# SajayR/TRIAD

Measured on AMD Instinct MI355X. Metric: tri-modal triples/sec (whole node) + loss parity, B=256 at 1/2/4/8 MI355X, higher is better.
Workload: dtype bf16

## Files before the change

include/triad_hip.h:

```cpp
#ifndef TRIAD_HIP_H
#define TRIAD_HIP_H

#include <hip/hip_runtime_api.h>

#ifdef __cplusplus
extern "C" {
#endif

#define TRIAD_EINVAL 1001

int triad_pairsim_nparts(int R_pad, int Bk);

int triad_pairsim_fwd(const void* Q, const void* K, int R, int R_pad, int Nq, int Bq, int Bk, int Nk_pad,
                      int Nk_eff, int D, const float* temp, float clamp_lo, int diag, int diag_off,
                      float* rowmax, int* argmax, double* nn_part, float* diagS, void* dS, long long CT,
                      double* st_part, const int* k_len, hipStream_t stream);

typedef struct triad_pairsim_problem {
  const void* Q;
  const void* K;
  int R, R_pad, Nq, Bq, Bk, Nk_pad, Nk_eff;
  const float* temp;
  float clamp_lo;
  int diag, diag_off;
// ... 161 lines not shown
                   hipStream_t stream);

long long triad_conv0_dw_workspace_bytes(int B, int T, int C);
int triad_conv0_dw(const void* wave, long long Lp, const void* dy0, int B, int T, int Tp, int C, void* ws, float* dw0,
                   hipStream_t stream);

int triad_posconv(const void* x, const void* wt, const float* bias, void* y, int B, int T, int C, int groups,
                  int pad, hipStream_t stream);

long long triad_posconv_dw_part_bytes(int C, int groups, int splits);
int triad_posconv_dw(const void* x, const void* dy, int B, int T, int C, int groups, int pad, int splits, float* part,
                     hipStream_t stream);

int triad_attn_fwd(const void* q, long long q_sB, long long q_sN, const void* k, long long k_sB, long long k_sN,
                   const void* v, long long v_sB, long long v_sN, int B, int H, int N, int D, float scale, void* out,
                   long long out_sB, long long out_sN, float* lse, hipStream_t stream);
int triad_attn_bwd(const void* q, long long q_sB, long long q_sN, const void* k, long long k_sB, long long k_sN,
                   const void* v, long long v_sB, long long v_sN, const void* o, long long o_sB, long long o_sN,
                   const void* dout, long long do_sB, long long do_sN, const float* lse, int B, int H, int N, int D,
                   float scale, void* dq, long long dq_sB, long long dq_sN, void* dk, long long dk_sB,
                   long long dk_sN, void* dv, long long dv_sB, long long dv_sN, float* delta, hipStream_t stream);
int triad_attn_dropmask(int B, int H, int N, float p, unsigned seed, unsigned* wq, unsigned* wk, hipStream_t stream);
int triad_attn_fwd_dropout(const void* q, long long q_sB, long long q_sN, const void* k, long long k_sB,
                           long long k_sN, const void* v, long long v_sB, long long v_sN, int B, int H, int N, int D,
                           float scale, const unsigned* wq, float p, void* out, long long out_sB, long long out_sN,
                           float* lse, hipStream_t stream);
int triad_attn_bwd_dropout(const void* q, long long q_sB, long long q_sN, const void* k, long long k_sB,
                           long long k_sN, const void* v, long long v_sB, long long v_sN, const void* o,
                           long long o_sB, long long o_sN, const void* dout, long long do_sB, long long do_sN,
                           const float* lse, int B, int H, int N, int D, float scale, const unsigned* wq,
                           const unsigned* wk, float p, void* dq, long long dq_sB, long long dq_sN, void* dk,
                           long long dk_sB, long long dk_sN, void* dv, long long dv_sB, long long dv_sN, float* delta,
                           hipStream_t stream);

int triad_attn_long_dropmask(int B, int H, int N, float p, unsigned seed, unsigned* wq, unsigned* wk,
                             hipStream_t stream);
int triad_attn_long_fwd(const void* q, long long q_sB, long long q_sN, const void* k, long long k_sB, long long k_sN,
                        const void* v, long long v_sB, long long v_sN, int B, int H, int N, int D, float scale,
                        const unsigned* wq, float p, void* out, long long out_sB, long long out_sN, float* lse,
                        hipStream_t stream);
int triad_attn_long_bwd(const void* q, long long q_sB, long long q_sN, const void* k, long long k_sB, long long k_sN,
                        const void* v, long long v_sB, long long v_sN, const void* o, long long o_sB, long long o_sN,
                        const void* dout, long long do_sB, long long do_sN, const float* lse, int B, int H, int N,
                        int D, float scale, const unsigned* wq, const unsigned* wk, float p, void* dq, long long dq_sB,
                        long long dq_sN, void* dk, long long dk_sB, long long dk_sN, void* dv, long long dv_sB,
                        long long dv_sN, float* delta, hipStream_t stream);

int triad_rows_nt(const void* X, long long ldx, int M, int K, const void* W, int J, void* out, hipStream_t stream);
int triad_lora_update(void* Y, long long ldy, int M, int O, const void* T, const void* Bs, hipStream_t stream);
int triad_lora_tn_blocks(int M);
int triad_lora_tn(const void* Y, long long ldy, int M, int O, const void* T, const void* Wt, void* dt, float alpha,
                  float* slabs, float* out, hipStream_t stream);

int triad_addln_fwd(const float* x, const void* y, const float* g, const float* w, const float* b, float eps, int M,
                    int D, float* xn, void* ln, int out_f32, float* mean, float* rstd, hipStream_t stream);
int triad_addln_bwd(const void* dln, int dln_f32, const float* dres, const float* xn, const float* mean,
                    const float* rstd, const float* w, const float* g, int M, int D, float* dx, void* dy,
                    hipStream_t stream);

int triad_dropaddln_fwd(const float* res, const void* y, const float* w, const float* b, float eps, int M, int D,
                        float p, unsigned seed, float* h, void* hb, float* mean, float* rstd, hipStream_t stream);
int triad_dropaddln_bwd_blocks(int M);
int triad_dropaddln_bwd(const float* dh, const void* dhb, const float* res, const void* y, const float* mean,
                        const float* rstd, const float* w, int M, int D, float p, unsigned seed, float* dres, void* dy,
                        float* part, hipStream_t stream);
long long triad_gelu_table_bytes(void);
// ... 23 lines not shown
```

triad_amd/_lib.py:

```python
from __future__ import annotations

import ctypes as C
import os
import threading

_HERE = os.path.dirname(os.path.abspath(__file__))
DEFAULT_LIB = os.path.join(_HERE, "libtriad_hip.so")
LIB_PATH = os.environ.get("TRIAD_LIB_VARIANT", DEFAULT_LIB)

vp, i32, u32, i64, f32, f64 = C.c_void_p, C.c_int, C.c_uint, C.c_longlong, C.c_float, C.c_double

SIGNATURES = {
    "triad_pairsim_nparts": [i32, i32],
    "triad_pairsim_fwd": [vp, vp, i32, i32, i32, i32, i32, i32, i32, i32, vp, f32, i32, i32, vp, vp, vp, vp, vp,
                          i64, vp, vp, vp],
    "triad_pairsim_fwd_multi": [vp, i32, vp],
    "triad_pairsim_diag": [vp, i32, vp],
    "triad_clip_reduce": [vp, i32, i32, i32, i32, vp, vp, vp, vp],
    "triad_diag_smooth": [vp, i32, i32, i32, i32, f64, vp, vp, vp, vp],
    "triad_diag_sparsity": [vp, i32, i32, i32, i32, f32, f64, vp, vp, vp, vp],
    "triad_losshead": [vp, i32, i32, vp, vp, i32, f64, vp, i32, f64, f32, vp, vp, vp, vp],
    "triad_pairsim_dS": [vp, vp, i32, i32, i32, i32, i32, i32, i32, i32, vp, f32, i32, i32, vp, vp, vp, vp, vp,
                         vp, i64, vp, vp],
    "triad_split_pack": [vp, i32, i32, i32, i64, vp, vp, vp],
# ... 43 lines not shown
    "triad_chgn_gelu_fwd": [vp, i32, i32, i32, i32, vp, vp, f32, vp, vp, vp, vp, vp],
    "triad_chgn_gelu_bwd": [vp, vp, i32, i32, i32, i32, vp, vp, vp, vp, vp, vp, vp, vp, vp],
    "triad_gemm_bf16_form": [vp, i64, i32, vp, i64, i32, i32, i32, i32, vp, vp, i64, i32, i32, vp],
    "triad_gemm_w8_workgroups": [i32, i32],
    "triad_gemm_bf16_tiles": [vp, i64, i32, vp, i64, i32, i32, i32, i32, vp, vp, i64, i32, vp, i32, i32, vp],
    "triad_conv0_dw_workspace_bytes": [i32, i32, i32],
    "triad_conv0_dw": [vp, i64, vp, i32, i32, i32, i32, vp, vp, vp],
    "triad_c0gn_fwd": [vp, i64, vp, i32, i32, i32, i32, vp, vp, f32, vp, vp, vp, vp, vp, vp],
    "triad_posconv": [vp, vp, vp, vp, i32, i32, i32, i32, i32, vp],
    "triad_posconv_dw_part_bytes": [i32, i32, i32],
    "triad_posconv_dw": [vp, vp, i32, i32, i32, i32, i32, i32, vp, vp],
    "triad_rows_nt": [vp, i64, i32, i32, vp, i32, vp, vp],
    "triad_lora_update": [vp, i64, i32, i32, vp, vp, vp],
    "triad_dropaddln_fwd": [vp, vp, vp, vp, f32, i32, i32, f32, u32, vp, vp, vp, vp, vp],
    "triad_dropaddln_bwd_blocks": [i32],
    "triad_dropaddln_bwd": [vp, vp, vp, vp, vp, vp, vp, i32, i32, f32, u32, vp, vp, vp, vp],
    "triad_gelu_table_bytes": [],
    "triad_gelu_table": [vp, vp],
    "triad_geludrop_fwd": [vp, i64, f32, u32, vp, vp, vp],
    "triad_geludrop_bwd": [vp, vp, i64, f32, u32, vp, vp, vp],
    "triad_dropout_keep": [i64, f32, u32, vp, vp],
    "triad_addln_fwd": [vp, vp, vp, vp, vp, f32, i32, i32, vp, vp, i32, vp, vp, vp],
    "triad_addln_bwd": [vp, i32, vp, vp, vp, vp, vp, vp, i32, i32, vp, vp, vp],
    "triad_lora_tn_blocks": [i32],
    "triad_lora_tn": [vp, i64, i32, i32, vp, vp, vp, f32, vp, vp, vp],
    "triad_attn_dropmask": [i32, i32, i32, f32, u32, vp, vp, vp],
    "triad_attn_fwd_dropout": [vp, i64, i64, vp, i64, i64, vp, i64, i64, i32, i32, i32, i32, f32, vp, f32, vp, i64,
                               i64, vp, vp],
    "triad_attn_bwd_dropout": [vp, i64, i64, vp, i64, i64, vp, i64, i64, vp, i64, i64, vp, i64, i64, vp, i32, i32,
                               i32, i32, f32, vp, vp, f32, vp, i64, i64, vp, i64, i64, vp, i64, i64, vp, vp],
    "triad_attn_fwd": [vp, i64, i64, vp, i64, i64, vp, i64, i64, i32, i32, i32, i32, f32, vp, i64, i64, vp, vp],
    "triad_attn_bwd": [vp, i64, i64, vp, i64, i64, vp, i64, i64, vp, i64, i64, vp, i64, i64, vp, i32, i32, i32,
                       i32, f32, vp, i64, i64, vp, i64, i64, vp, i64, i64, vp, vp],
    "triad_attn_long_dropmask": [i32, i32, i32, f32, u32, vp, vp, vp],
    "triad_attn_long_fwd": [vp, i64, i64, vp, i64, i64, vp, i64, i64, i32, i32, i32, i32, f32, vp, f32, vp, i64, i64,
                            vp, vp],
    "triad_attn_long_bwd": [vp, i64, i64, vp, i64, i64, vp, i64, i64, vp, i64, i64, vp, i64, i64, vp, i32, i32, i32,
                            i32, f32, vp, vp, f32, vp, i64, i64, vp, i64, i64, vp, i64, i64, vp, vp],
    "triad_dense_nparts": [i64],
    "triad_dense_rowmax": [vp, i32, i32, i32, i32, i32, vp, vp, vp],
    "triad_nonneg_fwd": [vp, i64, f32, vp, vp],
    "triad_nonneg_bwd": [vp, i64, f32, f32, vp, vp, vp],
    "triad_sims_bwd_pack": [vp, vp, vp, vp, vp, i32, i32, i32, i32, i32, vp, vp, i64, vp, vp],
    "triad_sum_parts": [vp, i32, f64, vp, vp],
}
RESTYPES = {"triad_pairsim_nparts": C.c_int, "triad_chgn_workspace_bytes": C.c_longlong,
            "triad_conv0_dw_workspace_bytes": C.c_longlong, "triad_gelu_table_bytes": C.c_longlong,
            "triad_posconv_dw_part_bytes": C.c_longlong,
            "triad_lora_tn_blocks": C.c_int, "triad_dropaddln_bwd_blocks": C.c_int,
            "triad_colsum_splits": C.c_int, "triad_colsum_dma_splits": C.c_int, "triad_dense_nparts": C.c_int,
            "triad_rowpanel_count": C.c_int, "triad_gemm_w8_workgroups": C.c_int}

BACKBONE_ENTRY_POINTS = frozenset({
    "triad_chgn_gelu_fwd", "triad_chgn_gelu_bwd", "triad_gemm_bf16_form", "triad_gemm_bf16_tiles", "triad_conv0_dw",
    "triad_c0gn_fwd",
    "triad_posconv", "triad_posconv_dw", "triad_gemm_bf16_splitk", "triad_rows_nt", "triad_lora_update",
    "triad_dropaddln_fwd", "triad_dropaddln_bwd", "triad_gelu_table", "triad_geludrop_fwd", "triad_geludrop_bwd",
    "triad_dropout_keep", "triad_addln_fwd", "triad_addln_bwd", "triad_lora_tn", "triad_attn_dropmask",
    "triad_attn_fwd_dropout", "triad_attn_bwd_dropout", "triad_attn_fwd", "triad_attn_bwd",
    "triad_attn_long_dropmask", "triad_attn_long_fwd", "triad_attn_long_bwd"})


def hot_path_entry_points():
    return tuple(n for n in SIGNATURES if n not in RESTYPES and n not in BACKBONE_ENTRY_POINTS)



class PairsimProblem(C.Structure):
    _fields_ = [("Q", vp), ("K", vp), ("R", i32), ("R_pad", i32), ("Nq", i32), ("Bq", i32), ("Bk", i32),
                ("Nk_pad", i32), ("Nk_eff", i32), ("temp", vp), ("clamp_lo", f32), ("diag", i32), ("diag_off", i32),
                ("rowmax", vp), ("argmax", vp), ("nn_part", vp), ("diagS", vp), ("dS", vp), ("CT", i64),
                ("st_part", vp), ("k_tiles", vp)]


_lock = threading.Lock()
_lib = None


class TriadError(RuntimeError):
    pass


def load():
    global _lib
    with _lock:
        if _lib is None:
            if not os.path.exists(LIB_PATH):
                raise TriadError(f"{LIB_PATH} not found: build it with `python -m triad_amd.build` "
                                 "(or __graft_entry__.build()); there is no CPU fallback")
            if LIB_PATH == DEFAULT_LIB:
                _check_fresh()
            lib = C.CDLL(LIB_PATH)
            for name, args in SIGNATURES.items():
# ... 68 lines not shown
```

triad_amd/csrc/attention.hip:

```cpp
#include "attention_tiles.h"

namespace {

template <int NT>
__device__ __forceinline__ void load_rows2(char* l0, const bf16* b0, long long s0, char* l1, const bf16* b1,
                                           long long s1, int N) {
  static_assert((NT * 32 * 8) % 256 == 0, "256 threads");
  constexpr int PER = NT * 32 * 8 / 256;
  bf16x8 r0[PER], r1[PER];
#pragma unroll
  for (int i = 0; i < PER; ++i) {
    const int e = threadIdx.x + 256 * i, r = e >> 3, c = e & 7;
    r0[i] = r < N ? *(const bf16x8*)(b0 + (long long)r * s0 + c * 8) : (bf16x8){};
    r1[i] = r < N ? *(const bf16x8*)(b1 + (long long)r * s1 + c * 8) : (bf16x8){};
  }
#pragma unroll
  for (int i = 0; i < PER; ++i) {
    const int e = threadIdx.x + 256 * i, r = e >> 3, c = e & 7;
    const int off = r * 128 + ((c ^ swz(r)) << 4);
    *(bf16x8*)(l0 + off) = r0[i];
    *(bf16x8*)(l1 + off) = r1[i];
  }
}

template <int NKT, bool DROP>
__global__ __launch_bounds__(256, 2) void attn_fwd_kernel(AttnArgs a) {
  __shared__ __attribute__((aligned(16))) char lds[2 * NKT * 32 * 128];
  char* kl = lds;
  char* vl = lds + NKT * 32 * 128;
  const int bh = blockIdx.y, b = bh / a.H, hh = bh - b * a.H;
  const int lane = threadIdx.x & 63, wave = threadIdx.x >> 6, h = lane >> 5, ql = lane & 31;
  const int qt = blockIdx.x * 4 + wave;
  const int q = qt * 32 + ql;
  const bool qok = q < a.N;
  bf16x8 qf[4];
  {
    const bf16* qp = a.q + b * a.q_sB + (long long)(qok ? q : 0) * a.q_sN + hh * HD + 8 * h;
#pragma unroll
    for (int s = 0; s < 4; ++s) qf[s] = qok ? *(const bf16x8*)(qp + 16 * s) : (bf16x8){};
  }
  load_rows2<NKT>(kl, a.k + b * a.k_sB + hh * HD, a.k_sN, vl, a.v + b * a.v_sB + hh * HD, a.v_sN, a.N);
  __syncthreads();
  if (qt * 32 >= a.N) return;
  f32x16 acc[NKT];
#pragma unroll
  for (int kt = 0; kt < NKT; ++kt) {
    acc[kt] = (f32x16){};
#pragma unroll
    for (int s = 0; s < 4; ++s) acc[kt] = mfma32(lds_b128(kl, kt * 32 + ql, 2 * s + h), qf[s], acc[kt]);
  }
  const int nlast = a.N - (NKT - 1) * 32;
  if (nlast < 32) {
#pragma unroll
    for (int v = 0; v < 16; ++v)
      if (acc_row(v, h) >= nlast) acc[NKT - 1][v] = -INFINITY;
  }
  float m = -INFINITY;
#pragma unroll
  for (int kt = 0; kt < NKT; ++kt)
#pragma unroll
    for (int v = 0; v < 16; ++v) m = fmaxf(m, acc[kt][v]);
  m = fmaxf(m, __shfl_xor(m, 32));
  const float c2 = a.scale * LOG2E;
  const float mo = m * c2;
  float l = 0.f;
#pragma unroll
  for (int kt = 0; kt < NKT; ++kt)
#pragma unroll
    for (int v = 0; v < 16; ++v) {
      const float p = __builtin_amdgcn_exp2f(fmaf(acc[kt][v], c2, -mo));
      acc[kt][v] = p;
      l += p;
    }
  l += __shfl_xor(l, 32);
  if (DROP) {
#pragma unroll
    for (int kt = 0; kt < NKT; ++kt) {
      const unsigned w = qok ? a.wq[((long long)bh * a.N + q) * NKT + kt] : 0u;
#pragma unroll
      for (int v = 0; v < 16; ++v) acc[kt][v] = tile_bit(w, v, h) ? acc[kt][v] : 0.f;
    }
  }

  f32x16 o0 = {}, o1 = {};
#pragma unroll
  for (int kt = 0; kt < NKT; ++kt)
#pragma unroll
    for (int half = 0; half < 2; ++half) {
      const int c = 2 * kt + half;
      const bf16x8 pf = pack8(acc[kt], half);
      o0 = mfma32(frag_tr(vl, c, 0, lane), pf, o0);
      o1 = mfma32(frag_tr(vl, c, 32, lane), pf, o1);
    }
  if (!qok) return;
  const float inv = (DROP ? a.drop_scale : 1.f) / l;
  bf16* op = a.out + b * a.out_sB + (long long)q * a.out_sN + hh * HD;
  store_cols(op, o0, inv, h);
  store_cols(op + 32, o1, inv, h);
  if (h == 0) a.lse[(long long)bh * a.N + q] = m * a.scale + logf(l);
}

template <int NKT, bool DROP>
__global__ __launch_bounds__(256, 2) void attn_dq_kernel(AttnArgs a) {
  __shared__ __attribute__((aligned(16))) char lds[2 * NKT * 32 * 128];
  char* kl = lds;
  char* vl = lds + NKT * 32 * 128;
  const int bh = blockIdx.y, b = bh / a.H, hh = bh - b * a.H;
  const int lane = threadIdx.x & 63, wave = threadIdx.x >> 6, h = lane >> 5, ql = lane & 31;
  const int qt = blockIdx.x * 4 + wave;
  const int q = qt * 32 + ql;
  const bool qok = q < a.N;
  bf16x8 qf[4], df[4], ov[4];
  {
    const long long qq = qok ? q : 0;
    const bf16* qp = a.q + b * a.q_sB + qq * a.q_sN + hh * HD + 8 * h;
    const bf16* dp = a.dout + b * a.do_sB + qq * a.do_sN + hh * HD + 8 * h;
    const bf16* op = a.o + b * a.o_sB + qq * a.o_sN + hh * HD + 8 * h;
#pragma unroll
    for (int s = 0; s < 4; ++s) {
      qf[s] = qok ? *(const bf16x8*)(qp + 16 * s) : (bf16x8){};
      df[s] = qok ? *(const bf16x8*)(dp + 16 * s) : (bf16x8){};
      ov[s] = qok ? *(const bf16x8*)(op + 16 * s) : (bf16x8){};
    }
  }
  const float lse2 = qok ? a.lse[(long long)bh * a.N + q] * LOG2E : 0.f;
  load_rows2<NKT>(kl, a.k + b * a.k_sB + hh * HD, a.k_sN, vl, a.v + b * a.v_sB + hh * HD, a.v_sN, a.N);
  __syncthreads();
  if (qt * 32 >= a.N) return;
  float dl = 0.f;
#pragma unroll
  for (int s = 0; s < 4; ++s)
#pragma unroll
    for (int i = 0; i < 8; ++i) dl = fmaf((float)df[s][i], (float)ov[s][i], dl);
  dl += __shfl_xor(dl, 32);
  if (qok && h == 0) a.delta[(long long)bh * a.N + q] = dl;
  const float c2 = a.scale * LOG2E;
  f32x16 g0 = {}, g1 = {};
#pragma unroll
  for (int kt = 0; kt < NKT; ++kt) {
    f32x16 s = {}, dp = {};
#pragma unroll
    for (int st = 0; st < 4; ++st) {
      s = mfma32(lds_b128(kl, kt * 32 + ql, 2 * st + h), qf[st], s);
      dp = mfma32(lds_b128(vl, kt * 32 + ql, 2 * st + h), df[st], dp);
    }
    const int nv = a.N - kt * 32;
    const unsigned w = DROP && qok ? a.wq[((long long)bh * a.N + q) * NKT + kt] : 0u;
#pragma unroll
    for (int v = 0; v < 16; ++v) {
      const bool ok = qok && acc_row(v, h) < nv;
      const float e = __builtin_amdgcn_exp2f(fmaf(s[v], c2, -lse2));
      const float p = ok ? e : 0.f;
      const float dpv = DROP ? (tile_bit(w, v, h) ? dp[v] * a.drop_scale : 0.f) : dp[v];
      s[v] = p * (dpv - dl);
    }
#pragma unroll
    for (int half = 0; half < 2; ++half) {
      const int c = 2 * kt + half;
      const bf16x8 sf = pack8(s, half);
      g0 = mfma32(frag_tr(kl, c, 0, lane), sf, g0);
      g1 = mfma32(frag_tr(kl, c, 32, lane), sf, g1);
    }
  }
  if (!qok) return;
  bf16* gp = a.dq + b * a.dq_sB + (long long)q * a.dq_sN + hh * HD;
  store_cols(gp, g0, a.scale, h);
  store_cols(gp + 32, g1, a.scale, h);
}

template <int NQT, bool DROP>
__global__ __launch_bounds__(256, 2) void attn_dkv_kernel(AttnArgs a) {
  __shared__ __attribute__((aligned(16))) char lds[2 * NQT * 32 * 128];
  __shared__ float stat[2][NQT * 32];
  char* ql_ = lds;
  char* dl_ = lds + NQT * 32 * 128;
  const int bh = blockIdx.y, b = bh / a.H, hh = bh - b * a.H;
  const int lane = threadIdx.x & 63, wave = threadIdx.x >> 6, h = lane >> 5, kl = lane & 31;
  const int kt = blockIdx.x * 4 + wave;
  const int key = kt * 32 + kl;
  const bool kok = key < a.N;
  bf16x8 kf[4], vf[4];
  {
    const long long kk = kok ? key : 0;
    const bf16* kp = a.k + b * a.k_sB + kk * a.k_sN + hh * HD + 8 * h;
    const bf16* vp = a.v + b * a.v_sB + kk * a.v_sN + hh * HD + 8 * h;
#pragma unroll
    for (int s = 0; s < 4; ++s) {
      kf[s] = kok ? *(const bf16x8*)(kp + 16 * s) : (bf16x8){};
      vf[s] = kok ? *(const bf16x8*)(vp + 16 * s) : (bf16x8){};
    }
  }
  load_rows2<NQT>(ql_, a.q + b * a.q_sB + hh * HD, a.q_sN, dl_, a.dout + b * a.do_sB + hh * HD, a.do_sN, a.N);
  for (int i = threadIdx.x; i < NQT * 32; i += blockDim.x) {
    const bool ok = i < a.N;
    stat[0][i] = ok ? a.lse[(long long)bh * a.N + i] * LOG2E : INFINITY;
    stat[1][i] = ok ? a.delta[(long long)bh * a.N + i] : 0.f;
  }
  __syncthreads();
  if (kt * 32 >= a.N) return;
  const float c2 = a.scale * LOG2E;
  f32x16 dv0 = {}, dv1 = {}, dk0 = {}, dk1 = {};
#pragma unroll 1
  for (int qt = 0; qt < NQT; ++qt) {
    f32x16 s = {}, dp = {};
#pragma unroll
    for (int st = 0; st < 4; ++st) {
      s = mfma32(lds_b128(ql_, qt * 32 + kl, 2 * st + h), kf[st], s);
      dp = mfma32(lds_b128(dl_, qt * 32 + kl, 2 * st + h), vf[st], dp);
    }
    const unsigned w = DROP && kok ? a.wk[((long long)bh * a.N + key) * NQT + qt] : 0u;
#pragma unroll
    for (int j = 0; j < 4; ++j) {
      const int q0 = qt * 32 + 8 * j + 4 * h;
      const f32x4 ls = *(const f32x4*)&stat[0][q0];
      const f32x4 de = *(const f32x4*)&stat[1][q0];
#pragma unroll
      for (int i = 0; i < 4; ++i) {
        const int v = 4 * j + i;
        const float e = __builtin_amdgcn_exp2f(fmaf(s[v], c2, -ls[i]));
        const float p = kok ? e : 0.f;
        if (DROP) {
          const float m = tile_bit(w, v, h) ? a.drop_scale : 0.f;
          s[v] = p * m;
          dp[v] = p * (dp[v] * m - de[i]);
        } else {
          s[v] = p;
          dp[v] = p * (dp[v] - de[i]);
        }
      }
    }
#pragma unroll
    for (int half = 0; half < 2; ++half) {
      const int c = 2 * qt + half;
      const bf16x8 pf = pack8(s, half);
      const bf16x8 sf = pack8(dp, half);
      const bf16x8 d0 = frag_tr(dl_, c, 0, lane), d1 = frag_tr(dl_, c, 32, lane);
      const bf16x8 q0 = frag_tr(ql_, c, 0, lane), q1 = frag_tr(ql_, c, 32, lane);
      dv0 = mfma32(pf, d0, dv0);
      dv1 = mfma32(pf, d1, dv1);
      dk0 = mfma32(sf, q0, dk0);
      dk1 = mfma32(sf, q1, dk1);
    }
  }
#pragma unroll
  for (int v = 0; v < 16; ++v) {
    const int kr = kt * 32 + acc_row(v, h);
    if (kr < a.N) {
      bf16* dkp = a.dk + b * a.dk_sB + (long long)kr * a.dk_sN + hh * HD + kl;
      bf16* dvp = a.dv + b * a.dv_sB + (long long)kr * a.dv_sN + hh * HD + kl;
      dkp[0] = (bf16)(dk0[v] * a.scale);
      dkp[32] = (bf16)(dk1[v] * a.scale);
      dvp[0] = (bf16)dv0[v];
      dvp[32] = (bf16)dv1[v];
    }
  }
}

#define ATTN_SWITCH(KERNEL, DR, NT, GRID, ARGS)                                                 \
  switch (NT) {                                                                                \
    case 1: hipLaunchKernelGGL((KERNEL<1, DR>), GRID, dim3(256), 0, stream, ARGS); break;       \
    case 2: hipLaunchKernelGGL((KERNEL<2, DR>), GRID, dim3(256), 0, stream, ARGS); break;       \
    case 3: hipLaunchKernelGGL((KERNEL<3, DR>), GRID, dim3(256), 0, stream, ARGS); break;       \
    case 4: hipLaunchKernelGGL((KERNEL<4, DR>), GRID, dim3(256), 0, stream, ARGS); break;       \
    case 5: hipLaunchKernelGGL((KERNEL<5, DR>), GRID, dim3(256), 0, stream, ARGS); break;       \
    case 6: hipLaunchKernelGGL((KERNEL<6, DR>), GRID, dim3(256), 0, stream, ARGS); break;       \
    case 7: hipLaunchKernelGGL((KERNEL<7, DR>), GRID, dim3(256), 0, stream, ARGS); break;       \
    case 8: hipLaunchKernelGGL((KERNEL<8, DR>), GRID, dim3(256), 0, stream, ARGS); break;       \
    case 9: hipLaunchKernelGGL((KERNEL<9, DR>), GRID, dim3(256), 0, stream, ARGS); break;       \
    default: hipLaunchKernelGGL((KERNEL<10, DR>), GRID, dim3(256), 0, stream, ARGS); break;     \
  }

static_assert(MAX_N_SHORT == 10 * 32, "ATTN_SWITCH instantiates 1 .. 10 tiles of 32");
}

extern "C" {

int triad_attn_fwd_dropout(const void* q, long long q_sB, long long q_sN, const void* k, long long k_sB,
                           long long k_sN, const void* v, long long v_sB, long long v_sN, int B, int H, int N, int D,
                           float scale, const unsigned* wq, float p, void* out, long long out_sB, long long out_sN,
                           float* lse, hipStream_t stream) {
  AttnArgs a = {};
  if (!attn_fwd_args(a, ATTN_SHORT, {q, q_sB, q_sN}, {k, k_sB, k_sN}, {v, v_sB, v_sN}, B, H, N, D, scale, wq, p,
                     {out, out_sB, out_sN}, lse))
    return TRIAD_EINVAL;
  const int nt = (N + 31) / 32;
  const dim3 grid = attn_grid(B, H, N);
  if (wq) { ATTN_SWITCH(attn_fwd_kernel, true, nt, grid, a) }
  else { ATTN_SWITCH(attn_fwd_kernel, false, nt, grid, a) }
  TRIAD_CHECK_LAUNCH();
  return TRIAD_OK;
}

int triad_attn_fwd(const void* q, long long q_sB, long long q_sN, const void* k, long long k_sB, long long k_sN,
                   const void* v, long long v_sB, long long v_sN, int B, int H, int N, int D, float scale, void* out,
                   long long out_sB, long long out_sN, float* lse, hipStream_t stream) {
  return triad_attn_fwd_dropout(q, q_sB, q_sN, k, k_sB, k_sN, v, v_sB, v_sN, B, H, N, D, scale, nullptr, 0.f, out,
                                out_sB, out_sN, lse, stream);
}

int triad_attn_bwd_dropout(const void* q, long long q_sB, long long q_sN, const void* k, long long k_sB,
                           long long k_sN, const void* v, long long v_sB, long long v_sN, const void* o,
                           long long o_sB, long long o_sN, const void* dout, long long do_sB, long long do_sN,
                           const float* lse, int B, int H, int N, int D, float scale, const unsigned* wq,
                           const unsigned* wk, float p, void* dq, long long dq_sB, long long dq_sN, void* dk,
                           long long dk_sB, long long dk_sN, void* dv, long long dv_sB, long long dv_sN, float* delta,
                           hipStream_t stream) {
  AttnArgs a = {};
  if (!attn_bwd_args(a, ATTN_SHORT, {q, q_sB, q_sN}, {k, k_sB, k_sN}, {v, v_sB, v_sN}, {o, o_sB, o_sN},
                     {dout, do_sB, do_sN}, lse, B, H, N, D, scale, wq, wk, p, {dq, dq_sB, dq_sN}, {dk, dk_sB, dk_sN},
                     {dv, dv_sB, dv_sN}, delta))
    return TRIAD_EINVAL;
  const int nt = (N + 31) / 32;
  const dim3 grid = attn_grid(B, H, N);
  if (wq) {
    ATTN_SWITCH(attn_dq_kernel, true, nt, grid, a)
    ATTN_SWITCH(attn_dkv_kernel, true, nt, grid, a)
  } else {
    ATTN_SWITCH(attn_dq_kernel, false, nt, grid, a)
    ATTN_SWITCH(attn_dkv_kernel, false, nt, grid, a)
  }
  TRIAD_CHECK_LAUNCH();
  return TRIAD_OK;
}

int triad_attn_bwd(const void* q, long long q_sB, long long q_sN, const void* k, long long k_sB, long long k_sN,
                   const void* v, long long v_sB, long long v_sN, const void* o, long long o_sB, long long o_sN,
                   const void* dout, long long do_sB, long long do_sN, const float* lse, int B, int H, int N, int D,
                   float scale, void* dq, long long dq_sB, long long dq_sN, void* dk, long long dk_sB,
                   long long dk_sN, void* dv, long long dv_sB, long long dv_sN, float* delta, hipStream_t stream) {
  return triad_attn_bwd_dropout(q, q_sB, q_sN, k, k_sB, k_sN, v, v_sB, v_sN, o, o_sB, o_sN, dout, do_sB, do_sN, lse,
                                B, H, N, D, scale, nullptr, nullptr, 0.f, dq, dq_sB, dq_sN, dk, dk_sB, dk_sN, dv,
                                dv_sB, dv_sN, delta, stream);
}

}
```

Measured before the change: 2066.

## Add one-block-per-head attention kernels that stage K/V once and loop over tiles

Adds head-form attention kernels (fwd, dq, dkv) where a single 256-thread block per (batch, head) stages K/V (or Q/dO) into LDS once and loops its four waves over all query/key tiles, prefetching the next tile's fragments. This replaces the per-tile grid in which every block reloaded the full K/V for its head. A per-kernel rule table chooses head form for sequences of five or more tiles, and it is on by default through the existing entry points. The cost is a smaller grid with less parallelism, which may underfill the GPU when B*H is small.

```diff
diff --git a/include/triad_hip.h b/include/triad_hip.h
--- a/include/triad_hip.h
+++ b/include/triad_hip.h
@@ -217,6 +217,17 @@
                            const unsigned* wk, float p, void* dq, long long dq_sB, long long dq_sN, void* dk,
                            long long dk_sB, long long dk_sN, void* dv, long long dv_sB, long long dv_sN, float* delta,
                            hipStream_t stream);
+int triad_attn_form(int kernel, int N);
+int triad_attn_fwd_form(const void* q, long long q_sB, long long q_sN, const void* k, long long k_sB, long long k_sN,
+                        const void* v, long long v_sB, long long v_sN, int B, int H, int N, int D, float scale,
+                        const unsigned* wq, float p, void* out, long long out_sB, long long out_sN, float* lse,
+                        int form, hipStream_t stream);
+int triad_attn_bwd_form(const void* q, long long q_sB, long long q_sN, const void* k, long long k_sB, long long k_sN,
+                        const void* v, long long v_sB, long long v_sN, const void* o, long long o_sB, long long o_sN,
+                        const void* dout, long long do_sB, long long do_sN, const float* lse, int B, int H, int N,
+                        int D, float scale, const unsigned* wq, const unsigned* wk, float p, void* dq, long long dq_sB,
+                        long long dq_sN, void* dk, long long dk_sB, long long dk_sN, void* dv, long long dv_sB,
+                        long long dv_sN, float* delta, int form, hipStream_t stream);
 
 int triad_attn_long_dropmask(int B, int H, int N, float p, unsigned seed, unsigned* wq, unsigned* wk,
                              hipStream_t stream);
diff --git a/triad_amd/_lib.py b/triad_amd/_lib.py
--- a/triad_amd/_lib.py
+++ b/triad_amd/_lib.py
@@ -99,6 +99,11 @@
     "triad_attn_fwd": [vp, i64, i64, vp, i64, i64, vp, i64, i64, i32, i32, i32, i32, f32, vp, i64, i64, vp, vp],
     "triad_attn_bwd": [vp, i64, i64, vp, i64, i64, vp, i64, i64, vp, i64, i64, vp, i64, i64, vp, i32, i32, i32,
                        i32, f32, vp, i64, i64, vp, i64, i64, vp, i64, i64, vp, vp],
+    "triad_attn_form": [i32, i32],
+    "triad_attn_fwd_form": [vp, i64, i64, vp, i64, i64, vp, i64, i64, i32, i32, i32, i32, f32, vp, f32, vp, i64, i64,
+                            vp, i32, vp],
+    "triad_attn_bwd_form": [vp, i64, i64, vp, i64, i64, vp, i64, i64, vp, i64, i64, vp, i64, i64, vp, i32, i32, i32,
+                            i32, f32, vp, vp, f32, vp, i64, i64, vp, i64, i64, vp, i64, i64, vp, i32, vp],
     "triad_attn_long_dropmask": [i32, i32, i32, f32, u32, vp, vp, vp],
     "triad_attn_long_fwd": [vp, i64, i64, vp, i64, i64, vp, i64, i64, i32, i32, i32, i32, f32, vp, f32, vp, i64, i64,
                             vp, vp],
@@ -116,7 +121,7 @@
             "triad_posconv_dw_part_bytes": C.c_longlong,
             "triad_lora_tn_blocks": C.c_int, "triad_dropaddln_bwd_blocks": C.c_int,
             "triad_colsum_splits": C.c_int, "triad_colsum_dma_splits": C.c_int, "triad_dense_nparts": C.c_int,
-            "triad_rowpanel_count": C.c_int, "triad_gemm_w8_workgroups": C.c_int}
+            "triad_rowpanel_count": C.c_int, "triad_gemm_w8_workgroups": C.c_int, "triad_attn_form": C.c_int}
 
 BACKBONE_ENTRY_POINTS = frozenset({
     "triad_chgn_gelu_fwd", "triad_chgn_gelu_bwd", "triad_gemm_bf16_form", "triad_gemm_bf16_tiles", "triad_conv0_dw",
@@ -125,7 +130,8 @@
     "triad_dropaddln_fwd", "triad_dropaddln_bwd", "triad_gelu_table", "triad_geludrop_fwd", "triad_geludrop_bwd",
     "triad_dropout_keep", "triad_addln_fwd", "triad_addln_bwd", "triad_lora_tn", "triad_attn_dropmask",
     "triad_attn_fwd_dropout", "triad_attn_bwd_dropout", "triad_attn_fwd", "triad_attn_bwd",
-    "triad_attn_long_dropmask", "triad_attn_long_fwd", "triad_attn_long_bwd"})
+    "triad_attn_fwd_form", "triad_attn_bwd_form", "triad_attn_long_dropmask", "triad_attn_long_fwd",
+    "triad_attn_long_bwd"})
 
 
 def hot_path_entry_points():
diff --git a/triad_amd/csrc/attention.hip b/triad_amd/csrc/attention.hip
--- a/triad_amd/csrc/attention.hip
+++ b/triad_amd/csrc/attention.hip
@@ -23,81 +23,162 @@
   }
 }
 
+
+__device__ __forceinline__ void fwd_frags(const AttnArgs& a, int b, int hh, int qt, int lane, bf16x8 (&qf)[4]) {
+  const int h = lane >> 5, q = qt * 32 + (lane & 31);
+  const bool qok = q < a.N;
+  const bf16* qp = a.q + b * a.q_sB + (long long)(qok ? q : 0) * a.q_sN + hh * HD + 8 * h;
+#pragma unroll
+  for (int s = 0; s < 4; ++s) qf[s] = qok ? *(const bf16x8*)(qp + 16 * s) : (bf16x8){};
+}
+
+template <int NKT, bool DROP>
+__device__ __forceinline__ void fwd_tile(const AttnArgs& a, const char* kl, const char* vl, int bh, int b, int hh,
+                                         int qt, int lane, const bf16x8 (&qf)[4]) {
+  const int h = lane >> 5, ql = lane & 31;
+  const int q = qt * 32 + ql;
+  const bool qok = q < a.N;
+  f32x16 acc[NKT];
+#pragma unroll
+  for (int kt = 0; kt < NKT; ++kt) {
+    acc[kt] = (f32x16){};
+#pragma unroll
+    for (int s = 0; s < 4; ++s) acc[kt] = mfma32(lds_b128(kl, kt * 32 + ql, 2 * s + h), qf[s], acc[kt]);
+  }
+  const int nlast = a.N - (NKT - 1) * 32;
+  if (nlast < 32) {
+#pragma unroll
+    for (int v = 0; v < 16; ++v)
+      if (acc_row(v, h) >= nlast) acc[NKT - 1][v] = -INFINITY;
+  }
+  float m = -INFINITY;
+#pragma unroll
+  for (int kt = 0; kt < NKT; ++kt)
+#pragma unroll
+    for (int v = 0; v < 16; ++v) m = fmaxf(m, acc[kt][v]);
+  m = fmaxf(m, __shfl_xor(m, 32));
+  const float c2 = a.scale * LOG2E;
+  const float mo = m * c2;
+  float l = 0.f;
+#pragma unroll
+  for (int kt = 0; kt < NKT; ++kt)
+#pragma unroll
+    for (int v = 0; v < 16; ++v) {
+      const float p = __builtin_amdgcn_exp2f(fmaf(acc[kt][v], c2, -mo));
+      acc[kt][v] = p;
+      l += p;
+    }
+  l += __shfl_xor(l, 32);
+  if (DROP) {
+#pragma unroll
+    for (int kt = 0; kt < NKT; ++kt) {
+      const unsigned w = qok ? a.wq[((long long)bh * a.N + q) * NKT + kt] : 0u;
+#pragma unroll
+      for (int v = 0; v < 16; ++v) acc[kt][v] = tile_bit(w, v, h) ? acc[kt][v] : 0.f;
+    }
+  }
+
+  f32x16 o0 = {}, o1 = {};
+#pragma unroll
+  for (int kt = 0; kt < NKT; ++kt)
+#pragma unroll
+    for (int half = 0; half < 2; ++half) {
+      const int c = 2 * kt + half;
+      const bf16x8 pf = pack8(acc[kt], half);
+      o0 = mfma32(frag_tr(vl, c, 0, lane), pf, o0);
+      o1 = mfma32(frag_tr(vl, c, 32, lane), pf, o1);
+    }
+  if (!qok) return;
+  const float inv = (DROP ? a.drop_scale : 1.f) / l;
+  bf16* op = a.out + b * a.out_sB + (long long)q * a.out_sN + hh * HD;
+  store_cols(op, o0, inv, h);
+  store_cols(op + 32, o1, inv, h);
+  if (h == 0) a.lse[(long long)bh * a.N + q] = m * a.scale + logf(l);
+}
+
 template <int NKT, bool DROP>
 __global__ __launch_bounds__(256, 2) void attn_fwd_kernel(AttnArgs a) {
   __shared__ __attribute__((aligned(16))) char lds[2 * NKT * 32 * 128];
   char* kl = lds;
   char* vl = lds + NKT * 32 * 128;
   const int bh = blockIdx.y, b = bh / a.H, hh = bh - b * a.H;
-  const int lane = threadIdx.x & 63, wave = threadIdx.x >> 6, h = lane >> 5, ql = lane & 31;
+  const int lane = threadIdx.x & 63, wave = threadIdx.x >> 6;
   const int qt = blockIdx.x * 4 + wave;
-  const int q = qt * 32 + ql;
-  const bool qok = q < a.N;
   bf16x8 qf[4];
-  {
-    const bf16* qp = a.q + b * a.q_sB + (long long)(qok ? q : 0) * a.q_sN + hh * HD + 8 * h;
-#pragma unroll
-    for (int s = 0; s < 4; ++s) qf[s] = qok ? *(const bf16x8*)(qp + 16 * s) : (bf16x8){};
-  }
+  fwd_frags(a, b, hh, qt, lane, qf);
   load_rows2<NKT>(kl, a.k + b * a.k_sB + hh * HD, a.k_sN, vl, a.v + b * a.v_sB + hh * HD, a.v_sN, a.N);
   __syncthreads();
   if (qt * 32 >= a.N) return;
-  f32x16 acc[NKT];
+  fwd_tile<NKT, DROP>(a, kl, vl, bh, b, hh, qt, lane, qf);
+}
+
+struct DqFrags {
+  bf16x8 qf[4], df[4], ov[4];
+  float lse2;
+};
+__device__ __forceinline__ void dq_frags(const AttnArgs& a, int bh, int b, int hh, int qt, int lane, DqFrags& f) {
+  const int h = lane >> 5, q = qt * 32 + (lane & 31);
+  const bool qok = q < a.N;
+  const long long qq = qok ? q : 0;
+  const bf16* qp = a.q + b * a.q_sB + qq * a.q_sN + hh * HD + 8 * h;
+  const bf16* dp = a.dout + b * a.do_sB + qq * a.do_sN + hh * HD + 8 * h;
+  const bf16* op = a.o + b * a.o_sB + qq * a.o_sN + hh * HD + 8 * h;
+#pragma unroll
+  for (int s = 0; s < 4; ++s) {
+    f.qf[s] = qok ? *(const bf16x8*)(qp + 16 * s) : (bf16x8){};
+    f.df[s] = qok ? *(const bf16x8*)(dp + 16 * s) : (bf16x8){};
+    f.ov[s] = qok ? *(const bf16x8*)(op + 16 * s) : (bf16x8){};
+  }
+  f.lse2 = qok ? a.lse[(long long)bh * a.N + q] * LOG2E : 0.f;
+}
+
+template <int NKT, bool DROP>
+__device__ __forceinline__ void dq_tile(const AttnArgs& a, const char* kl, const char* vl, int bh, int b, int hh,
+                                        int qt, int lane, const DqFrags& f) {
+  const int h = lane >> 5, ql = lane & 31;
+  const int q = qt * 32 + ql;
+  const bool qok = q < a.N;
+  const bf16x8 (&qf)[4] = f.qf, (&df)[4] = f.df, (&ov)[4] = f.ov;
+  const float lse2 = f.lse2;
+  float dl = 0.f;
+#pragma unroll
+  for (int s = 0; s < 4; ++s)
+#pragma unroll
+    for (int i = 0; i < 8; ++i) dl = fmaf((float)df[s][i], (float)ov[s][i], dl);
+  dl += __shfl_xor(dl, 32);
+  if (qok && h == 0) a.delta[(long long)bh * a.N + q] = dl;
+  const float c2 = a.scale * LOG2E;
+  f32x16 g0 = {}, g1 = {};
 #pragma unroll
   for (int kt = 0; kt < NKT; ++kt) {
-    acc[kt] = (f32x16){};
-#pragma unroll
-    for (int s = 0; s < 4; ++s) acc[kt] = mfma32(lds_b128(kl, kt * 32 + ql, 2 * s + h), qf[s], acc[kt]);
-  }
-  const int nlast = a.N - (NKT - 1) * 32;
-  if (nlast < 32) {
-#pragma unroll
-    for (int v = 0; v < 16; ++v)
-      if (acc_row(v, h) >= nlast) acc[NKT - 1][v] = -INFINITY;
-  }
-  float m = -INFINITY;
-#pragma unroll
-  for (int kt = 0; kt < NKT; ++kt)
-#pragma unroll
-    for (int v = 0; v < 16; ++v) m = fmaxf(m, acc[kt][v]);
-  m = fmaxf(m, __shfl_xor(m, 32));
-  const float c2 = a.scale * LOG2E;
-  const float mo = m * c2;
-  float l = 0.f;
-#pragma unroll
-  for (int kt = 0; kt < NKT; ++kt)
+    f32x16 s = {}, dp = {};
+#pragma unroll
+    for (int st = 0; st < 4; ++st) {
+      s = mfma32(lds_b128(kl, kt * 32 + ql, 2 * st + h), qf[st], s);
+      dp = mfma32(lds_b128(vl, kt * 32 + ql, 2 * st + h), df[st], dp);
+    }
+    const int nv = a.N - kt * 32;
+    const unsigned w = DROP && qok ? a.wq[((long long)bh * a.N + q) * NKT + kt] : 0u;
 #pragma unroll
     for (int v = 0; v < 16; ++v) {
-      const float p = __builtin_amdgcn_exp2f(fmaf(acc[kt][v], c2, -mo));
-      acc[kt][v] = p;
-      l += p;
-    }
-  l += __shfl_xor(l, 32);
-  if (DROP) {
-#pragma unroll
-    for (int kt = 0; kt < NKT; ++kt) {
-      const unsigned w = qok ? a.wq[((long long)bh * a.N + q) * NKT + kt] : 0u;
-#pragma unroll
-      for (int v = 0; v < 16; ++v) acc[kt][v] = tile_bit(w, v, h) ? acc[kt][v] : 0.f;
-    }
-  }
-
-  f32x16 o0 = {}, o1 = {};
-#pragma unroll
-  for (int kt = 0; kt < NKT; ++kt)
+      const bool ok = qok && acc_row(v, h) < nv;
+      const float e = __builtin_amdgcn_exp2f(fmaf(s[v], c2, -lse2));
+      const float p = ok ? e : 0.f;
+      const float dpv = DROP ? (tile_bit(w, v, h) ? dp[v] * a.drop_scale : 0.f) : dp[v];
+      s[v] = p * (dpv - dl);
+    }
 #pragma unroll
     for (int half = 0; half < 2; ++half) {
       const int c = 2 * kt + half;
-      const bf16x8 pf = pack8(acc[kt], half);
-      o0 = mfma32(frag_tr(vl, c, 0, lane), pf, o0);
-      o1 = mfma32(frag_tr(vl, c, 32, lane), pf, o1);
-    }
+      const bf16x8 sf = pack8(s, half);
+      g0 = mfma32(frag_tr(kl, c, 0, lane), sf, g0);
+      g1 = mfma32(frag_tr(kl, c, 32, lane), sf, g1);
+    }
+  }
   if (!qok) return;
-  const float inv = (DROP ? a.drop_scale : 1.f) / l;
-  bf16* op = a.out + b * a.out_sB + (long long)q * a.out_sN + hh * HD;
-  store_cols(op, o0, inv, h);
-  store_cols(op + 32, o1, inv, h);
-  if (h == 0) a.lse[(long long)bh * a.N + q] = m * a.scale + logf(l);
+  bf16* gp = a.dq + b * a.dq_sB + (long long)q * a.dq_sN + hh * HD;
+  store_cols(gp, g0, a.scale, h);
+  store_cols(gp + 32, g1, a.scale, h);
 }
 
 template <int NKT, bool DROP>
@@ -106,98 +187,51 @@
   char* kl = lds;
   char* vl = lds + NKT * 32 * 128;
   const int bh = blockIdx.y, b = bh / a.H, hh = bh - b * a.H;
-  const int lane = threadIdx.x & 63, wave = threadIdx.x >> 6, h = lane >> 5, ql = lane & 31;
+  const int lane = threadIdx.x & 63, wave = threadIdx.x >> 6;
   const int qt = blockIdx.x * 4 + wave;
-  const int q = qt * 32 + ql;
-  const bool qok = q < a.N;
-  bf16x8 qf[4], df[4], ov[4];
-  {
-    const long long qq = qok ? q : 0;
-    const bf16* qp = a.q + b * a.q_sB + qq * a.q_sN + hh * HD + 8 * h;
-    const bf16* dp = a.dout + b * a.do_sB + qq * a.do_sN + hh * HD + 8 * h;
-    const bf16* op = a.o + b * a.o_sB + qq * a.o_sN + hh * HD + 8 * h;
-#pragma unroll
-    for (int s = 0; s < 4; ++s) {
-      qf[s] = qok ? *(const bf16x8*)(qp + 16 * s) : (bf16x8){};
-      df[s] = qok ? *(const bf16x8*)(dp + 16 * s) : (bf16x8){};
-      ov[s] = qok ? *(const bf16x8*)(op + 16 * s) : (bf16x8){};
-    }
-  }
-  const float lse2 = qok ? a.lse[(long long)bh * a.N + q] * LOG2E : 0.f;
+  DqFrags f;
+  dq_frags(a, bh, b, hh, qt, lane, f);
   load_rows2<NKT>(kl, a.k + b * a.k_sB + hh * HD, a.k_sN, vl, a.v + b * a.v_sB + hh * HD, a.v_sN, a.N);
   __syncthreads();
   if (qt * 32 >= a.N) return;
-  float dl = 0.f;
-#pragma unroll
-  for (int s = 0; s < 4; ++s)
-#pragma unroll
-    for (int i = 0; i < 8; ++i) dl = fmaf((float)df[s][i], (float)ov[s][i], dl);
-  dl += __shfl_xor(dl, 32);
-  if (qok && h == 0) a.delta[(long long)bh * a.N + q] = dl;
-  const float c2 = a.scale * LOG2E;
-  f32x16 g0 = {}, g1 = {};
-#pragma unroll
-  for (int kt = 0; kt < NKT; ++kt) {
-    f32x16 s = {}, dp = {};
-#pragma unroll
-    for (int st = 0; st < 4; ++st) {
-      s = mfma32(lds_b128(kl, kt * 32 + ql, 2 * st + h), qf[st], s);
-      dp = mfma32(lds_b128(vl, kt * 32 + ql, 2 * st + h), df[st], dp);
-    }
-    const int nv = a.N - kt * 32;
-    const unsigned w = DROP && qok ? a.wq[((long long)bh * a.N + q) * NKT + kt] : 0u;
-#pragma unroll
-    for (int v = 0; v < 16; ++v) {
-      const bool ok = qok && acc_row(v, h) < nv;
-      const float e = __builtin_amdgcn_exp2f(fmaf(s[v], c2, -lse2));
-      const float p = ok ? e : 0.f;
-      const float dpv = DROP ? (tile_bit(w, v, h) ? dp[v] * a.drop_scale : 0.f) : dp[v];
-      s[v] = p * (dpv - dl);
-    }
-#pragma unroll
-    for (int half = 0; half < 2; ++half) {
-      const int c = 2 * kt + half;
-      const bf16x8 sf = pack8(s, half);
-      g0 = mfma32(frag_tr(kl, c, 0, lane), sf, g0);
-      g1 = mfma32(frag_tr(kl, c, 32, lane), sf, g1);
-    }
-  }
-  if (!qok) return;
-  bf16* gp = a.dq + b * a.dq_sB + (long long)q * a.dq_sN + hh * HD;
-  store_cols(gp, g0, a.scale, h);
-  store_cols(gp + 32, g1, a.scale, h);
-}
-
-template <int NQT, bool DROP>
-__global__ __launch_bounds__(256, 2) void attn_dkv_kernel(AttnArgs a) {
-  __shared__ __attribute__((aligned(16))) char lds[2 * NQT * 32 * 128];
-  __shared__ float stat[2][NQT * 32];
-  char* ql_ = lds;
-  char* dl_ = lds + NQT * 32 * 128;
-  const int bh = blockIdx.y, b = bh / a.H, hh = bh - b * a.H;
-  const int lane = threadIdx.x & 63, wave = threadIdx.x >> 6, h = lane >> 5, kl = lane & 31;
-  const int kt = blockIdx.x * 4 + wave;
-  const int key = kt * 32 + kl;
+  dq_tile<NKT, DROP>(a, kl, vl, bh, b, hh, qt, lane, f);
+}
+
+struct DkvFrags {
+  bf16x8 kf[4], vf[4];
+};
+__device__ __forceinline__ void dkv_frags(const AttnArgs& a, int b, int hh, int kt, int lane, DkvFrags& f) {
+  const int h = lane >> 5, key = kt * 32 + (lane & 31);
   const bool kok = key < a.N;
-  bf16x8 kf[4], vf[4];
-  {
-    const long long kk = kok ? key : 0;
-    const bf16* kp = a.k + b * a.k_sB + kk * a.k_sN + hh * HD + 8 * h;
-    const bf16* vp = a.v + b * a.v_sB + kk * a.v_sN + hh * HD + 8 * h;
-#pragma unroll
-    for (int s = 0; s < 4; ++s) {
-      kf[s] = kok ? *(const bf16x8*)(kp + 16 * s) : (bf16x8){};
-      vf[s] = kok ? *(const bf16x8*)(vp + 16 * s) : (bf16x8){};
-    }
-  }
+  const long long kk = kok ? key : 0;
+  const bf16* kp = a.k + b * a.k_sB + kk * a.k_sN + hh * HD + 8 * h;
+  const bf16* vp = a.v + b * a.v_sB + kk * a.v_sN + hh * HD + 8 * h;
+#pragma unroll
+  for (int s = 0; s < 4; ++s) {
+    f.kf[s] = kok ? *(const bf16x8*)(kp + 16 * s) : (bf16x8){};
+    f.vf[s] = kok ? *(const bf16x8*)(vp + 16 * s) : (bf16x8){};
+  }
+}
+
+template <int NQT>
+__device__ __forceinline__ void dkv_stage(const AttnArgs& a, int bh, int b, int hh, char* ql_, char* dl_,
+                                          float (&stat)[2][NQT * 32]) {
   load_rows2<NQT>(ql_, a.q + b * a.q_sB + hh * HD, a.q_sN, dl_, a.dout + b * a.do_sB + hh * HD, a.do_sN, a.N);
   for (int i = threadIdx.x; i < NQT * 32; i += blockDim.x) {
     const bool ok = i < a.N;
     stat[0][i] = ok ? a.lse[(long long)bh * a.N + i] * LOG2E : INFINITY;
     stat[1][i] = ok ? a.delta[(long long)bh * a.N + i] : 0.f;
   }
-  __syncthreads();
-  if (kt * 32 >= a.N) return;
+}
+
+template <int NQT, bool DROP>
+__device__ __forceinline__ void dkv_tile(const AttnArgs& a, const char* ql_, const char* dl_,
+                                         const float (&stat)[2][NQT * 32], int bh, int b, int hh, int kt, int lane,
+                                         const DkvFrags& f) {
+  const int h = lane >> 5, kl = lane & 31;
+  const int key = kt * 32 + kl;
+  const bool kok = key < a.N;
+  const bf16x8 (&kf)[4] = f.kf, (&vf)[4] = f.vf;
   const float c2 = a.scale * LOG2E;
   f32x16 dv0 = {}, dv1 = {}, dk0 = {}, dk1 = {};
 #pragma unroll 1
@@ -256,6 +290,112 @@
   }
 }
 
+template <int NQT, bool DROP>
+__global__ __launch_bounds__(256, 2) void attn_dkv_kernel(AttnArgs a) {
+  __shared__ __attribute__((aligned(16))) char lds[2 * NQT * 32 * 128];
+  __shared__ float stat[2][NQT * 32];
+  char* ql_ = lds;
+  char* dl_ = lds + NQT * 32 * 128;
+  const int bh = blockIdx.y, b = bh / a.H, hh = bh - b * a.H;
+  const int lane = threadIdx.x & 63, wave = threadIdx.x >> 6;
+  const int kt = blockIdx.x * 4 + wave;
+  DkvFrags f;
+  dkv_frags(a, b, hh, kt, lane, f);
+  dkv_stage<NQT>(a, bh, b, hh, ql_, dl_, stat);
+  __syncthreads();
+  if (kt * 32 >= a.N) return;
+  dkv_tile<NQT, DROP>(a, ql_, dl_, stat, bh, b, hh, kt, lane, f);
+}
+
+#ifndef TRIAD_ATTN_HEAD_ROTATE
+#define TRIAD_ATTN_HEAD_ROTATE 1
+#endif
+#ifndef TRIAD_ATTN_HEAD_PREFETCH
+#define TRIAD_ATTN_HEAD_PREFETCH 1
+#endif
+constexpr bool HEAD_ROTATE = TRIAD_ATTN_HEAD_ROTATE;
+constexpr bool HEAD_PREFETCH = TRIAD_ATTN_HEAD_PREFETCH;
+
+__device__ __forceinline__ void head_tile_fence(int& lane) { asm volatile("" : "+v"(lane) : : "memory"); }
+
+__device__ __forceinline__ int head_first_tile(int wave, int bh) { return HEAD_ROTATE ? (wave + bh) & 3 : wave; }
+
+template <int NKT, bool DROP>
+__global__ __launch_bounds__(256, 2) void attn_fwd_head_kernel(AttnArgs a) {
+  static_assert(NKT > 4, "NT <= 4 is one workgroup per head in the one-tile grid");
+  __shared__ __attribute__((aligned(16))) char lds[2 * NKT * 32 * 128];
+  char* kl = lds;
+  char* vl = lds + NKT * 32 * 128;
+  const int bh = blockIdx.y, b = bh / a.H, hh = bh - b * a.H;
+  int lane = threadIdx.x & 63;
+  const int wave = threadIdx.x >> 6;
+  int qt = head_first_tile(wave, bh);
+  bf16x8 qf[4];
+  fwd_frags(a, b, hh, qt, lane, qf);
+  load_rows2<NKT>(kl, a.k + b * a.k_sB + hh * HD, a.k_sN, vl, a.v + b * a.v_sB + hh * HD, a.v_sN, a.N);
+  __syncthreads();
+  constexpr bool PREFETCH = HEAD_PREFETCH && !(DROP && NKT == 10);
+#pragma unroll 1
+  for (; qt < NKT; qt += 4) {
+    head_tile_fence(lane);
+    if (PREFETCH) {
+      bf16x8 nx[4];
+      fwd_frags(a, b, hh, qt + 4, lane, nx);
+      fwd_tile<NKT, DROP>(a, kl, vl, bh, b, hh, qt, lane, qf);
+#pragma unroll
+      for (int s = 0; s < 4; ++s) qf[s] = nx[s];
+    } else {
+      fwd_tile<NKT, DROP>(a, kl, vl, bh, b, hh, qt, lane, qf);
+      fwd_frags(a, b, hh, qt + 4, lane, qf);
+    }
+  }
+}
+
+template <int NKT, bool DROP>
+__global__ __launch_bounds__(256, 2) void attn_dq_head_kernel(AttnArgs a) {
+  static_assert(NKT > 4, "NT <= 4 is one workgroup per head in the one-tile grid");
+  __shared__ __attribute__((aligned(16))) char lds[2 * NKT * 32 * 128];
+  char* kl = lds;
+  char* vl = lds + NKT * 32 * 128;
+  const int bh = blockIdx.y, b = bh / a.H, hh = bh - b * a.H;
+  int lane = threadIdx.x & 63;
+  const int wave = threadIdx.x >> 6;
+  int qt = head_first_tile(wave, bh);
+  DqFrags f;
+  dq_frags(a, bh, b, hh, qt, lane, f);
+  load_rows2<NKT>(kl, a.k + b * a.k_sB + hh * HD, a.k_sN, vl, a.v + b * a.v_sB + hh * HD, a.v_sN, a.N);
+  __syncthreads();
+#pragma unroll 1
+  for (; qt < NKT; qt += 4) {
+    head_tile_fence(lane);
+    dq_tile<NKT, DROP>(a, kl, vl, bh, b, hh, qt, lane, f);
+    dq_frags(a, bh, b, hh, qt + 4, lane, f);
+  }
+}
+
+template <int NQT, bool DROP>
+__global__ __launch_bounds__(256, 2) void attn_dkv_head_kernel(AttnArgs a) {
+  static_assert(NQT > 4, "NT <= 4 is one workgroup per head in the one-tile grid");
+  __shared__ __attribute__((aligned(16))) char lds[2 * NQT * 32 * 128];
+  __shared__ float stat[2][NQT * 32];
+  char* ql_ = lds;
+  char* dl_ = lds + NQT * 32 * 128;
+  const int bh = blockIdx.y, b = bh / a.H, hh = bh - b * a.H;
+  int lane = threadIdx.x & 63;
+  const int wave = threadIdx.x >> 6;
+  int kt = head_first_tile(wave, bh);
+  DkvFrags f;
+  dkv_frags(a, b, hh, kt, lane, f);
+  dkv_stage<NQT>(a, bh, b, hh, ql_, dl_, stat);
+  __syncthreads();
+#pragma unroll 1
+  for (; kt < NQT; kt += 4) {
+    head_tile_fence(lane);
+    dkv_tile<NQT, DROP>(a, ql_, dl_, stat, bh, b, hh, kt, lane, f);
+    dkv_frags(a, b, hh, kt + 4, lane, f);
+  }
+}
+
 #define ATTN_SWITCH(KERNEL, DR, NT, GRID, ARGS)                                                 \
   switch (NT) {                                                                                \
     case 1: hipLaunchKernelGGL((KERNEL<1, DR>), GRID, dim3(256), 0, stream, ARGS); break;       \
@@ -271,24 +411,73 @@
   }
 
 static_assert(MAX_N_SHORT == 10 * 32, "ATTN_SWITCH instantiates 1 .. 10 tiles of 32");
+
+#define ATTN_HEAD_SWITCH(KERNEL, DR, NT, GRID, ARGS)                                            \
+  switch (NT) {                                                                                \
+    case 5: hipLaunchKernelGGL((KERNEL<5, DR>), GRID, dim3(256), 0, stream, ARGS); break;       \
+    case 6: hipLaunchKernelGGL((KERNEL<6, DR>), GRID, dim3(256), 0, stream, ARGS); break;       \
+    case 7: hipLaunchKernelGGL((KERNEL<7, DR>), GRID, dim3(256), 0, stream, ARGS); break;       \
+    case 8: hipLaunchKernelGGL((KERNEL<8, DR>), GRID, dim3(256), 0, stream, ARGS); break;       \
+    case 9: hipLaunchKernelGGL((KERNEL<9, DR>), GRID, dim3(256), 0, stream, ARGS); break;       \
+    default: hipLaunchKernelGGL((KERNEL<10, DR>), GRID, dim3(256), 0, stream, ARGS); break;     \
+  }
+
+enum { ATTN_FWD = 0, ATTN_DQ = 1, ATTN_DKV = 2 };
+constexpr int ATTN_HEAD_MIN_NT = 5;
+constexpr unsigned char ATTN_RULE[3][6] = {
+    {2, 2, 2, 2, 2, 2},
+    {2, 2, 2, 2, 2, 2},
+    {2, 2, 1, 2, 1, 2},
+};
+#ifndef TRIAD_ATTN_RULE_FORCE
+#define TRIAD_ATTN_RULE_FORCE 0
+#endif
+inline int attn_rule(int kernel, int nt) {
+  if (nt < ATTN_HEAD_MIN_NT) return 1;
+  return (TRIAD_ATTN_RULE_FORCE >> kernel) & 1 ? 2 : ATTN_RULE[kernel][nt - ATTN_HEAD_MIN_NT];
+}
+inline bool attn_form_ok(int form) { return form >= 0 && form <= 2; }
+inline bool attn_head(int form, int kernel, int nt) {
+  return nt >= ATTN_HEAD_MIN_NT && (form ? form : attn_rule(kernel, nt)) == 2;
+}
 }
 
 extern "C" {
+
+int triad_attn_form(int kernel, int N) {
+  if (kernel < ATTN_FWD || kernel > ATTN_DKV || N < 1 || N > MAX_N_SHORT) return 0;
+  return attn_rule(kernel, (N + 31) / 32);
+}
+
+int triad_attn_fwd_form(const void* q, long long q_sB, long long q_sN, const void* k, long long k_sB, long long k_sN,
+                        const void* v, long long v_sB, long long v_sN, int B, int H, int N, int D, float scale,
+                        const unsigned* wq, float p, void* out, long long out_sB, long long out_sN, float* lse,
+                        int form, hipStream_t stream) {
+  AttnArgs a = {};
+  if (!attn_form_ok(form) ||
+      !attn_fwd_args(a, ATTN_SHORT, {q, q_sB, q_sN}, {k, k_sB, k_sN}, {v, v_sB, v_sN}, B, H, N, D, scale, wq, p,
+                     {out, out_sB, out_sN}, lse))
+    return TRIAD_EINVAL;
+  const int nt = (N + 31) / 32;
+  if (attn_head(form, ATTN_FWD, nt)) {
+    const dim3 grid(1, B * H);
+    if (wq) { ATTN_HEAD_SWITCH(attn_fwd_head_kernel, true, nt, grid, a) }
+    else { ATTN_HEAD_SWITCH(attn_fwd_head_kernel, false, nt, grid, a) }
+  } else {
+    const dim3 grid = attn_grid(B, H, N);
+    if (wq) { ATTN_SWITCH(attn_fwd_kernel, true, nt, grid, a) }
+    else { ATTN_SWITCH(attn_fwd_kernel, false, nt, grid, a) }
+  }
+  TRIAD_CHECK_LAUNCH();
+  return TRIAD_OK;
+}
 
 int triad_attn_fwd_dropout(const void* q, long long q_sB, long long q_sN, const void* k, long long k_sB,
                            long long k_sN, const void* v, long long v_sB, long long v_sN, int B, int H, int N, int D,
                            float scale, const unsigned* wq, float p, void* out, long long out_sB, long long out_sN,
                            float* lse, hipStream_t stream) {
-  AttnArgs a = {};
-  if (!attn_fwd_args(a, ATTN_SHORT, {q, q_sB, q_sN}, {k, k_sB, k_sN}, {v, v_sB, v_sN}, B, H, N, D, scale, wq, p,
-                     {out, out_sB, out_sN}, lse))
-    return TRIAD_EINVAL;
-  const int nt = (N + 31) / 32;
-  const dim3 grid = attn_grid(B, H, N);
-  if (wq) { ATTN_SWITCH(attn_fwd_kernel, true, nt, grid, a) }
-  else { ATTN_SWITCH(attn_fwd_kernel, false, nt, grid, a) }
-  TRIAD_CHECK_LAUNCH();
-  return TRIAD_OK;
+  return triad_attn_fwd_form(q, q_sB, q_sN, k, k_sB, k_sN, v, v_sB, v_sN, B, H, N, D, scale, wq, p, out, out_sB,
+                             out_sN, lse, 0, stream);
 }
 
 int triad_attn_fwd(const void* q, long long q_sB, long long q_sN, const void* k, long long k_sB, long long k_sN,
@@ -296,6 +485,38 @@
                    long long out_sB, long long out_sN, float* lse, hipStream_t stream) {
   return triad_attn_fwd_dropout(q, q_sB, q_sN, k, k_sB, k_sN, v, v_sB, v_sN, B, H, N, D, scale, nullptr, 0.f, out,
                                 out_sB, out_sN, lse, stream);
+}
+
+int triad_attn_bwd_form(const void* q, long long q_sB, long long q_sN, const void* k, long long k_sB, long long k_sN,
+                        const void* v, long long v_sB, long long v_sN, const void* o, long long o_sB, long long o_sN,
+                        const void* dout, long long do_sB, long long do_sN, const float* lse, int B, int H, int N,
+                        int D, float scale, const unsigned* wq, const unsigned* wk, float p, void* dq, long long dq_sB,
+                        long long dq_sN, void* dk, long long dk_sB, long long dk_sN, void* dv, long long dv_sB,
+                        long long dv_sN, float* delta, int form, hipStream_t stream) {
+  AttnArgs a = {};
+  if (!attn_form_ok(form) ||
+      !attn_bwd_args(a, ATTN_SHORT, {q, q_sB, q_sN}, {k, k_sB, k_sN}, {v, v_sB, v_sN}, {o, o_sB, o_sN},
+                     {dout, do_sB, do_sN}, lse, B, H, N, D, scale, wq, wk, p, {dq, dq_sB, dq_sN}, {dk, dk_sB, dk_sN},
+                     {dv, dv_sB, dv_sN}, delta))
+    return TRIAD_EINVAL;
+  const int nt = (N + 31) / 32;
+  const dim3 tiles = attn_grid(B, H, N), heads(1, B * H);
+  if (attn_head(form, ATTN_DQ, nt)) {
+    if (wq) { ATTN_HEAD_SWITCH(attn_dq_head_kernel, true, nt, heads, a) }
+    else { ATTN_HEAD_SWITCH(attn_dq_head_kernel, false, nt, heads, a) }
+  } else {
+    if (wq) { ATTN_SWITCH(attn_dq_kernel, true, nt, tiles, a) }
+    else { ATTN_SWITCH(attn_dq_kernel, false, nt, tiles, a) }
+  }
+  if (attn_head(form, ATTN_DKV, nt)) {
+    if (wq) { ATTN_HEAD_SWITCH(attn_dkv_head_kernel, true, nt, heads, a) }
+    else { ATTN_HEAD_SWITCH(attn_dkv_head_kernel, false, nt, heads, a) }
+  } else {
+    if (wq) { ATTN_SWITCH(attn_dkv_kernel, true, nt, tiles, a) }
+    else { ATTN_SWITCH(attn_dkv_kernel, false, nt, tiles, a) }
+  }
+  TRIAD_CHECK_LAUNCH();
+  return TRIAD_OK;
 }
 
 int triad_attn_bwd_dropout(const void* q, long long q_sB, long long q_sN, const void* k, long long k_sB,
@@ -305,22 +526,9 @@
                            const unsigned* wk, float p, void* dq, long long dq_sB, long long dq_sN, void* dk,
                            long long dk_sB, long long dk_sN, void* dv, long long dv_sB, long long dv_sN, float* delta,
                            hipStream_t stream) {
-  AttnArgs a = {};
-  if (!attn_bwd_args(a, ATTN_SHORT, {q, q_sB, q_sN}, {k, k_sB, k_sN}, {v, v_sB, v_sN}, {o, o_sB, o_sN},
-                     {dout, do_sB, do_sN}, lse, B, H, N, D, scale, wq, wk, p, {dq, dq_sB, dq_sN}, {dk, dk_sB, dk_sN},
-                     {dv, dv_sB, dv_sN}, delta))
-    return TRIAD_EINVAL;
-  const int nt = (N + 31) / 32;
-  const dim3 grid = attn_grid(B, H, N);
-  if (wq) {
-    ATTN_SWITCH(attn_dq_kernel, true, nt, grid, a)
-    ATTN_SWITCH(attn_dkv_kernel, true, nt, grid, a)
-  } else {
-    ATTN_SWITCH(attn_dq_kernel, false, nt, grid, a)
-    ATTN_SWITCH(attn_dkv_kernel, false, nt, grid, a)
-  }
-  TRIAD_CHECK_LAUNCH();
-  return TRIAD_OK;
+  return triad_attn_bwd_form(q, q_sB, q_sN, k, k_sB, k_sN, v, v_sB, v_sN, o, o_sB, o_sN, dout, do_sB, do_sN, lse, B, H,
+                             N, D, scale, wq, wk, p, dq, dq_sB, dq_sN, dk, dk_sB, dk_sN, dv, dv_sB, dv_sN, delta, 0,
+                             stream);
 }
 
 int triad_attn_bwd(const void* q, long long q_sB, long long q_sN, const void* k, long long k_sB, long long k_sN,
```

New measurement: 2076 (median of 6 runs). About the same (+0.5%).
